# madsjulia/GeostatInversion.jl

Measured on AMD Instinct MI355X. Metric: randSVD GB/s + top-k singular-value rel-err, n=1e6 rank=256, higher is better.
Workload: dtype f64

## Files before the change

### geostatinversion.jl_amd/context.py

```python
import ctypes as C

import numpy as np

from . import _lib as L


class Context:

    def __init__(self, device=0, lib=None):
        self.lib = lib or L.load()
        h = C.c_void_p()
        L.check(self.lib.gsi_ctx_create(C.byref(h), int(device)), self.lib)
        self.h = h
        self.device = int(device)
        self._children = []

    def close(self):
        if getattr(self, "h", None):
            for ch in list(self._children):
                ch.close()
            self.lib.gsi_ctx_destroy(self.h)
            self.h = None

    def __del__(self):
# ... 42 lines not shown

    def phase_times(self):
        ms = (C.c_double * len(L.PHASES))()
        cnt = (C.c_int64 * len(L.PHASES))()
        L.check(self.lib.gsi_ctx_phase_times(self.h, ms, cnt), self.lib)
        return {name: (ms[i], cnt[i]) for i, name in enumerate(L.PHASES)}

    def counters(self):
        out = (C.c_int64 * 4)()
        L.check(self.lib.gsi_ctx_counters(self.h, out), self.lib)
        return {"cholqr2": out[0], "householder": out[1], "jacobi_sweeps": out[2], "scholqr3": out[3]}

    LU_FORMS = ["none", "replicated", "per-step", "persistent-1hop", "persistent-2hop", "persistent-ov"]

    def path_info(self):
        n = 16
        out = (C.c_int64 * n)()
        L.check(self.lib.gsi_ctx_path_info(self.h, out, n), self.lib)
        forms = {self.LU_FORMS[f]: int(out[6 + f]) for f in range(1, 6) if out[6 + f]}
        return {"lu_form": self.LU_FORMS[out[0]] if 0 <= out[0] < 6 else int(out[0]), "lu_forms_run": forms,
                "lu_selftest_mask": int(out[1]), "collectives": int(out[2]), "n_ranks_seen": int(out[3]),
                "lu_timeouts": int(out[4]), "lu_timeouts_recovered": int(out[5]), "svd_sweep_cap_hits": int(out[12]),
                "lowrank_tails": int(out[13]), "lowrank_power_steps": int(out[14]), "lowrank_power_declines": int(out[15])}

    def release_cache(self):
        L.check(self.lib.gsi_ctx_release_cache(self.h), self.lib)

    def device_bytes(self):
        b = C.c_int64()
        L.check(self.lib.gsi_ctx_device_bytes(self.h, C.byref(b)), self.lib)
        return b.value


class _Handle:
    _destroy = None

    def __init__(self, ctx, h):
        self.ctx, self.h = ctx, h
# ... 180 lines not shown
```

### geostatinversion.jl_amd/csrc/api.cpp

```cpp
#include <cmath>
#include <cstdlib>
#include <cstring>
#include <memory>
#include <new>
#include <string>
#include <vector>
#include "../../include/gsi_hip.h"
#include "pipeline.hpp"
#include "pointcov.hpp"

using namespace gsi;

struct gsi_ctx {
  Context c;
};
struct gsi_op {
  Operator op;
};
struct gsi_mat {
  gsi_ctx* ctx;
  Buf buf;
  int64_t rows, cols;
  int refs = 1;
};
// ... 151 lines not shown
  return guarded([&] {
    REQUIRE(ctx && out && n_out >= 1, "bad argument");
    Context& c = ctx->c;
    int64_t v[GSI_PATH_INFO_COUNT] = {0};
    v[GSI_PATH_LU_FORM_LAST] = c.lu_form_last;
    v[GSI_PATH_LU_SELFTEST_MASK] = c.lus_mr_selftest;
    v[GSI_PATH_COLLECTIVES] = c.comm ? c.comm->ncollectives : 0;
    v[GSI_PATH_RANKS_SEEN] = c.ranks_seen;
    v[GSI_PATH_LU_TIMEOUTS] = c.be->lu_timeouts();
    v[GSI_PATH_LU_TIMEOUTS_RECOVERED] = c.lu_timeouts_recovered;
    for (int f = 0; f < (int)Context::LU_FORMS; ++f) v[GSI_PATH_LU_FORM_COUNTS + f] = c.lu_form_count[f];
    v[GSI_PATH_SVD_CAP_HITS] = c.be->svd_cap_hits();
    v[GSI_PATH_LOWRANK_TAILS] = c.lowrank_tails;
    v[GSI_PATH_LOWRANK_POWER_STEPS] = c.lowrank_power_steps;
    v[GSI_PATH_LOWRANK_POWER_DECLINES] = c.lowrank_power_declines;
    for (int64_t i = 0; i < n_out; ++i) out[i] = i < GSI_PATH_INFO_COUNT ? v[i] : 0;
  });
}

int gsi_ctx_pinned_copy_rate(gsi_ctx* ctx, int64_t bytes, double* h2d_gbs, double* d2h_gbs) {
  return guarded([&] {
    REQUIRE(ctx && h2d_gbs && d2h_gbs, "NULL argument");
    REQUIRE(bytes >= 0 && bytes <= ((int64_t)64 << 30), "bad size");
    ctx->c.be->pinned_copy_rate(bytes, h2d_gbs, d2h_gbs);
  });
}

int gsi_ctx_rank(gsi_ctx* ctx, int* rank, int* nranks) {
  return guarded([&] {
    REQUIRE(ctx, "ctx is NULL");
// ... 1053 lines not shown
```

### geostatinversion.jl_amd/csrc/backend.hpp

```cpp
#pragma once
#include <cstddef>
#include <cstdint>
#include <stdexcept>
#include <string>

namespace gsi {

struct Error : std::runtime_error {
  int code;
  Error(int c, const std::string& msg) : std::runtime_error(msg), code(c) {}
};

enum Phase : int {
  PH_GEMM_N = 0, PH_GEMM_T = 1, PH_LU = 2, PH_QR = 3, PH_SVD = 4, PH_SMALL_GEMM = 5,
  PH_COMM = 6, PH_OTHER = 7, PH_COMM_WAIT = 8, PH_COUNT = 9
};

class Backend {
 public:
  virtual ~Backend() {}
  virtual const char* name() const = 0;

  virtual double* alloc(size_t count) = 0;
  virtual void release(double* p) = 0;
// ... 95 lines not shown
  }
  virtual bool sample_gram(const double* S, int64_t ld, int64_t n, int64_t N, double* G) {
    (void)S; (void)ld; (void)n; (void)N; (void)G;
    return false;
  }
  virtual bool lowrank_tail(const double* S, int64_t lds, int64_t n, int64_t N, const double* G, const double* T, int64_t l,
                            int64_t K, double c, double* Z, int64_t ldz, double* Sv) {
    (void)S; (void)lds; (void)n; (void)N; (void)G; (void)T; (void)l; (void)K; (void)c; (void)Z; (void)ldz; (void)Sv;
    return false;
  }
  virtual bool lowrank_power_step(const double* S, int64_t lds, int64_t n, int64_t N, const double* G, const double* T,
                                  const int32_t* ipiv, const double* L, int64_t ldl, int64_t l, double c, double* T_next) {
    (void)S; (void)lds; (void)n; (void)N; (void)G; (void)T; (void)ipiv; (void)L; (void)ldl; (void)l; (void)c; (void)T_next;
    return false;
  }
  virtual void svd_small(double* G, int64_t l, double* U, double* S) = 0;
  virtual void chol_upper(double* B, int64_t j) = 0;
  virtual void trsm_right_upper(double* F, int64_t m, int64_t j, int64_t ldf, const double* C) = 0;

  virtual void scale_cols_sqrt(double* U, int64_t l, const double* S, int64_t K) = 0;
  virtual void center_rows(double* S, int64_t n, int64_t N, int64_t ld) = 0;
  virtual void randn(double* p, size_t count, uint64_t seed) = 0;
  virtual void fill_gridcov(double* A, int64_t lda, int64_t nx, int64_t ny, double ell, int kind,
                            int64_t row0, int64_t mloc) = 0;
  virtual void fill_lowrank_samples(double* S, int64_t ld, int64_t nloc, int64_t N, int64_t row0, uint64_t seed,
                                    double decay) = 0;
  virtual void fftrf_fields(double* dst, int64_t ldd, int64_t row0, int64_t nloc, int64_t nf, int ndims, const int64_t* N,
                            double k0, double dk, double beta, const double* phi, int64_t ldphi, uint64_t seed,
                            int64_t field0) {
    (void)dst; (void)ldd; (void)row0; (void)nloc; (void)nf; (void)ndims; (void)N; (void)k0; (void)dk; (void)beta; (void)phi;
// ... 21 lines not shown
  virtual void lsqr_step_v(int64_t n, const double* t, double* v, double* w, double* x, double* work) = 0;

  virtual void f64_to_f32(const double* src, void* dst32, size_t count) = 0;
  virtual void pcga_params_f32(const void* Z32, int64_t n, int64_t K, const double* s, const double* X, double delta,
                               double* out) = 0;
  virtual void basis_gemv_f32(const void* Z32, int64_t n, int64_t K, const double* w, double beta, const double* X,
                              double* y) = 0;

  virtual int take_error(std::string* msg) = 0;
  virtual bool retryable_failure() { return false; }
  virtual void forgive_lost_coresidency() {}

  virtual void profile(bool on) = 0;
  virtual void phase_begin(Phase p) = 0;
  virtual void phase_end(Phase p) = 0;
  virtual void phase_reset() = 0;
  virtual void phase_times(double* ms, int64_t* counts) = 0;
  virtual void counters(int64_t* out4) { out4[0] = out4[1] = out4[2] = out4[3] = 0; }
  virtual int64_t lu_timeouts() { return 0; }
  virtual int64_t svd_cap_hits() { return 0; }
  virtual void set_ranks_sharing_device(int n) { (void)n; }
};

class Comm {
 public:
  int rank = 0, nranks = 1;
  int64_t ncollectives = 0;
  virtual ~Comm() {}
  void allreduce_sum(double* buf, size_t count) { ++ncollectives; do_allreduce_sum(buf, count); }
  void allgather(const double* send, double* recv, size_t count) { ++ncollectives; do_allgather(send, recv, count); }
// ... 8 lines not shown
  virtual void do_allgather(const double* send, double* recv, size_t count) = 0;
  virtual void do_reduce_scatter_sum(const double* send, double* recv, size_t count) = 0;
  virtual void do_alltoall(const double* send, double* recv, size_t count) = 0;
};

Backend* make_backend(int device_id);
Comm* make_comm(Backend* be, int nranks, int rank, const void* unique_id);
void comm_unique_id(void* id_out);
const char* backend_name();

struct ScopedPhase {
  Backend* be; Phase p;
  ScopedPhase(Backend* b, Phase ph) : be(b), p(ph) { be->phase_begin(p); }
  ~ScopedPhase() { be->phase_end(p); }
};

}
```

### geostatinversion.jl_amd/csrc/hip_backend.hip

```cpp
#include <hip/hip_runtime.h>
#include <rccl/rccl.h>
#include <dlfcn.h>
#include <fcntl.h>
#include <sched.h>
#include <sys/mman.h>
#include <time.h>
#include <unistd.h>
#include <algorithm>
#include <cmath>
#include <cstdlib>
#include <cstring>
#include <condition_variable>
#include <atomic>
#include <mutex>
#include <string>
#include <chrono>
#include <map>
#include <memory>
#include <set>
#include <vector>
#include "../../include/gsi_hip.h"
#include "backend.hpp"
#include "hip_common.hpp"
#include "host_staging.hpp"
// ... 45 lines not shown
    HIP_CHECK(hipGetDeviceProperties(&prop, device_));
    arch_ = prop.gcnArchName;
    ncus_ = prop.multiProcessorCount;
    if (arch_.find("gfx950") == std::string::npos)
      throw Error(GSI_ERR_HIP, "libgsi_hip is built for gfx950 (MI355X); device reports " + arch_);
    HIP_CHECK(hipStreamCreateWithFlags(&st_, hipStreamNonBlocking));
    HIP_CHECK(hipMalloc(&flags_, 16 * sizeof(int32_t)));
    HIP_CHECK(hipMemsetAsync(flags_, 0, 16 * sizeof(int32_t), st_));
    HIP_CHECK(hipMalloc(&scal_, (64 + 8 + 256) * sizeof(double)));
  }
  ~HipBackend() override {
    hipSetDevice(device_);
    hipStreamSynchronize(st_);
    stager_.reset();
    if (ev_stage_) hipEventDestroy(ev_stage_);
    for (auto& b : {&ws_gemm_, &ws_lu_, &ws_qr_, &ws_svd_, &ws_blas2_, &ws_lus_, &ws_svdf_, &ws_qr_hh_}) free_ws(*b);
    collect_garbage();
    for (auto& b : pool_) hipFree(b.p);
    for (auto& ev : ev_pool_) hipEventDestroy(ev);
    for (auto& r : records_) { hipEventDestroy(r.a); hipEventDestroy(r.b); }
    hipFree(flags_);
    hipFree(scal_);
    if (pin_power_) hipHostFree(pin_power_);
    if (mr_recs_) hipFree(mr_recs_);
    hipStreamDestroy(st_);
  }
  const char* name() const override { return "hip-gfx950"; }
  hipStream_t stream() const { return st_; }
  void bind() { hipSetDevice(device_); }

  double* alloc(size_t count) override {
// ... 56 lines not shown
    }
    const int64_t cap = ((int64_t)160 << 30) / std::max(1, ranks_sharing_device_);
    if (pooled_ > cap) trim_pool(cap / 3 * 2);
  }
  void trim_pool(int64_t keep_bytes) {
    hipStreamSynchronize(st_);
    std::lock_guard<std::mutex> g(mu_);
    while (!pool_.empty() && pooled_ > keep_bytes) {
      hipFree(pool_.back().p);
      pooled_ -= (int64_t)pool_.back().bytes;
      pool_.pop_back();
    }
  }
  void release_cache() override {
    bind();
    for (DevBuf* b : {&ws_gemm_, &ws_lu_, &ws_qr_, &ws_svd_, &ws_blas2_, &ws_lus_, &ws_svdf_, &ws_qr_hh_})
      if (b->bytes > ((size_t)64 << 20)) free_ws(*b);
    (void)hipStreamSynchronize(st_);
    collect_garbage();
    trim_pool(0);
  }
  int64_t bytes_in_use() const override {
    int64_t ws = 0;
    for (const DevBuf* b : {&ws_gemm_, &ws_lu_, &ws_qr_, &ws_svd_, &ws_blas2_, &ws_svdf_, &ws_qr_hh_})
      if (!b->pooled) ws += (int64_t)b->bytes;
    return in_use_ + pooled_ + ws + (int64_t)garbage_bytes_;
  }
  HostStager* stager() {
    if (stager_ || stager_failed_) return stager_.get();
    static const int threads = getenv("GSI_STAGE_THREADS") ? std::max(1, std::min(32, atoi(getenv("GSI_STAGE_THREADS")))) : 6;
    static const size_t chunk = (size_t)(getenv("GSI_STAGE_CHUNK_MB") ? std::max(1, std::min(1024, atoi(getenv("GSI_STAGE_CHUNK_MB")))) : 16) << 20;
    try {
      stager_.reset(new HostStager(device_, threads, chunk));
      HIP_CHECK(hipEventCreateWithFlags(&ev_stage_, hipEventDisableTiming));
    } catch (const std::exception&) {
      (void)hipGetLastError();
      stager_.reset();
      stager_failed_ = true;
    }
// ... 845 lines not shown
    const Verdict* h = static_cast<const Verdict*>(pin_power_);
    HIP_CHECK(hipMemcpyAsync(pin_power_, part, sizeof(Verdict), hipMemcpyDeviceToHost, st_));
    HIP_CHECK(hipStreamSynchronize(st_));
    double mx = 0.0;
    bool finite = true;
    for (int p = 0; p < NPARTS; ++p) {
      if (!std::isfinite(h->parts[p])) finite = false;
      else mx = std::max(mx, h->parts[p]);
    }
    if (!finite) mx = INFINITY;
    if (trace) fprintf(stderr, "lowrank_power_step: n %lld N %lld l %lld, %lld moved rows, check max |(P S) C - L| = %.3e\n",
                       (long long)n, (long long)N, (long long)l, (long long)h->v[2], mx);
    if (h->v[0] != 0 || h->v[1] != 0) return false;
    return finite && mx <= CHECK_MAX;
  }
  void svd_small(double* G, int64_t l, double* U, double* S) override {
    bind();
    if (l > 5000) throw Error(GSI_ERR_ARG, "sketch width l = K+p > 5000 is not supported by the LDS-resident block Jacobi SVD");
    grow(ws_svd_, sizeof(double) * (l + 8) + 64 + sizeof(int32_t) * hipk::SVD_SCHED_INTS);
    hipk::SvdWork w;
    w.norms = (double*)ws_svd_.p;
    w.pairs = (int32_t*)((char*)ws_svd_.p + sizeof(double) * (l + 8) + 64);
    w.rotcount = flags_ + 8;
    const int sw = hipk::svd_small(st_, G, l, U, S, w);
    last_svd_sweeps_ = sw < 0 ? -sw : sw;
    if (sw < 0) ++n_svd_cap_hits_;
    check_launch("svd_small");
  }
  void chol_upper(double* B, int64_t j) override {
    bind();
// ... 198 lines not shown
      return GSI_ERR_NOT_POSDEF;
    }
    return 0;
  }

  void profile(bool on) override { prof_ = on; }
  void phase_begin(Phase p) override {
    if (!prof_) return;
    bind();
    if (roctx().push) roctx().push(kPhaseNames[p]);
    cur_.phase = p;
    cur_.a = get_event();
    cur_.b = get_event();
    hipEventRecord(cur_.a, st_);
  }
  void phase_end(Phase) override {
    if (!prof_) return;
    if (roctx().pop) roctx().pop();
    hipEventRecord(cur_.b, st_);
    records_.push_back(cur_);
  }
  void phase_reset() override {
    bind();
    hipStreamSynchronize(st_);
    for (auto& r : records_) { ev_pool_.push_back(r.a); ev_pool_.push_back(r.b); }
    records_.clear();
    for (int i = 0; i < PH_COUNT; ++i) { acc_ms_[i] = 0.0; acc_n_[i] = 0; }
  }
  void phase_times(double* ms, int64_t* counts) override {
    bind();
    hipStreamSynchronize(st_);
    for (auto& r : records_) {
      float t = 0.f;
      if (hipEventElapsedTime(&t, r.a, r.b) == hipSuccess) { acc_ms_[r.phase] += t; acc_n_[r.phase] += 1; }
      ev_pool_.push_back(r.a);
      ev_pool_.push_back(r.b);
    }
    records_.clear();
    for (int i = 0; i < PH_COUNT; ++i) { ms[i] = acc_ms_[i]; counts[i] = acc_n_[i]; }
  }

  void counters(int64_t* out4) override {
    out4[0] = n_cholqr_; out4[1] = n_householder_; out4[2] = last_svd_sweeps_; out4[3] = n_scholqr3_;
  }
  int64_t lu_timeouts() override { return n_lu_timeouts_; }
  int64_t svd_cap_hits() override { return n_svd_cap_hits_; }
  void set_ranks_sharing_device(int n) override { ranks_sharing_device_ = n; }
  int device() const { return device_; }

 private:
  struct Scratch {
    HipBackend* be; double* p;
    Scratch(HipBackend* b, size_t doubles) : be(b), p(doubles ? b->alloc(doubles) : nullptr) {}
    ~Scratch() { if (p) be->release(p); }
    Scratch(const Scratch&) = delete;
    Scratch& operator=(const Scratch&) = delete;
  };
  struct Rec { Phase phase; hipEvent_t a, b; };
  hipEvent_t get_event() {
    if (!ev_pool_.empty()) { hipEvent_t e = ev_pool_.back(); ev_pool_.pop_back(); return e; }
    hipEvent_t e;
    hipEventCreate(&e);
    return e;
  }
  void check_launch(const char* what) {
    hipError_t e = hipGetLastError();
    if (e != hipSuccess) throw Error(GSI_ERR_HIP, std::string(what) + ": " + hipGetErrorString(e));
  }
  void free_ws(DevBuf& b) {
    if (!b.p) return;
    if (b.pooled) release((double*)b.p);
    else { std::lock_guard<std::mutex> g(mu_); garbage_.push_back(b.p); garbage_bytes_ += b.bytes; }
    b.p = nullptr; b.bytes = 0; b.pooled = false;
// ... 38 lines not shown
    if (doubles == 0) return (double*)ws_gemm_.p;
    grow(ws_gemm_, doubles * sizeof(double));
    return (double*)ws_gemm_.p;
  }

  int device_;
  int ncus_ = 0;
  std::string arch_;
  hipStream_t st_ = nullptr;
  std::unique_ptr<HostStager> stager_;
  bool stager_failed_ = false;
  hipEvent_t ev_stage_ = nullptr;
  int32_t* flags_ = nullptr;
  double* scal_ = nullptr;
  void* pin_power_ = nullptr;
  DevBuf ws_gemm_, ws_lu_, ws_qr_, ws_svd_, ws_blas2_, ws_lus_, ws_svdf_, ws_qr_hh_;
  std::mutex mu_;
  std::vector<DevBuf> sizes_;
  std::vector<DevBuf> pool_;
  std::vector<void*> garbage_;
  size_t garbage_bytes_ = 0;
  int64_t in_use_ = 0, pooled_ = 0;
  bool prof_ = false;
  Rec cur_{};
  std::vector<Rec> records_;
  std::vector<hipEvent_t> ev_pool_;
  double acc_ms_[PH_COUNT] = {0};
  int64_t acc_n_[PH_COUNT] = {0};
  int last_svd_sweeps_ = 0;
  int64_t n_svd_cap_hits_ = 0;
  int64_t n_cholqr_ = 0, n_householder_ = 0, n_scholqr3_ = 0;
// ... 470 lines not shown
```

### geostatinversion.jl_amd/csrc/hip_common.hpp

```cpp
#pragma once
#include <hip/hip_runtime.h>
#include <atomic>
#include <cstdint>
#include <cstddef>
#include "pointcov.hpp"

namespace gsi { namespace hipk {

inline bool first_use_on_this_device(std::atomic<uint64_t>& mask) {
  int dev = 0;
  if (hipGetDevice(&dev) != hipSuccess || dev < 0 || dev > 63) return true;
  const uint64_t bit = (uint64_t)1 << dev;
  return (mask.fetch_or(bit, std::memory_order_acq_rel) & bit) == 0;
}

struct GemmPlan { int64_t nt, nchunks, xmode, wide, nsplit, persistent, grid_x, active; };
size_t gemm_workspace_doubles(int64_t M, int64_t L, int64_t K);
void gemm_f64(hipStream_t st, bool transA, int64_t M, int64_t L, int64_t K, double alpha, const double* A,
              int64_t lda, const double* B, int64_t ldb, double beta, double* C, int64_t ldc, double* ws,
              GemmPlan* plan = nullptr);
size_t gemm_rowblock_workspace_doubles(int64_t M_full, int64_t mb, int64_t L, int64_t K);
void gemm_f64_nn_rowblock(hipStream_t st, int64_t M_full, int64_t r0, int64_t mb, int64_t L, int64_t K, const double* A,
                          int64_t lda, const double* B, int64_t ldb, double* C, int64_t ldc, double* ws,
                          GemmPlan* plan = nullptr);
// ... 144 lines not shown
void tri_product(hipStream_t st, const double* R2, const double* R1, int64_t l, double* R);
bool tri_inverse(hipStream_t st, const double* R, int64_t l, double* X);
void lr_gather_rows(hipStream_t st, const double* S, int64_t lds, int64_t N, const int64_t* src, const int64_t* sub,
                    int64_t nr, double* R, int64_t ldr);
void lr_check_rows(hipStream_t st, const double* E, int64_t lde, const double* L, int64_t ldl, const int64_t* rows,
                   int64_t nchk, int64_t l, double* part, int nparts);
void scholqr3_factor(hipStream_t st, const double* Y, int64_t m, int64_t l, int64_t ld, double* T, int64_t ldt,
                     double* S, int64_t lds, double* small_ws, int32_t* flag, double* gemm_ws);
void scholqr3_apply(hipStream_t st, double* Y, int64_t m, int64_t l, int64_t ld, const double* S, int64_t lds,
                    double* R, double* small_ws, double* gemm_ws);

void lr_compose(hipStream_t st, const int32_t* piv, const int32_t* info, int64_t n, int64_t l, int64_t nchk, int64_t o_chk,
                int64_t o_sm, int64_t ldr, int64_t* src, int64_t* sub, int64_t* chk, int32_t* verdict);
void lr_solve_u(hipStream_t st, const double* L, int64_t ldl, const double* Mp, int64_t l, double c, double* Ut);
void lr_solve_c(hipStream_t st, const double* Ut, int64_t l, const double* T, int64_t N, double c, double* C);
struct SvdWork {
  int32_t* rotcount;
  double* norms;
  int32_t* pairs;
};
constexpr int SVD_SCHED_INTS = 4096;
int svd_small(hipStream_t st, double* G, int64_t l, double* U, double* S, const SvdWork& w);

void center_rows(hipStream_t st, double* S, int64_t n, int64_t N, int64_t ld);
void scale_cols_sqrt(hipStream_t st, double* U, int64_t l, const double* S, int64_t K);
void randn_fill(hipStream_t st, double* p, size_t count, uint64_t seed);
void fill_gridcov(hipStream_t st, double* A, int64_t lda, int64_t nx, int64_t ny, double ell, int kind,
                  int64_t row0, int64_t mloc);
void fill_lowrank_samples(hipStream_t st, double* S, int64_t ld, int64_t nloc, int64_t N, int64_t row0, uint64_t seed,
                          double decay);
// ... 25 lines not shown
```

### geostatinversion.jl_amd/csrc/lowrank_power.hip

```cpp
#include "hip_common.hpp"
#include <climits>

namespace gsi { namespace hipk {

constexpr int LRP_MAXL = 384;
constexpr int LRP_THREADS = 256;
constexpr int LRP_ITEMS = 3;

constexpr int LRP_PER = (LRP_MAXL + LRP_THREADS - 1) / LRP_THREADS;

__global__ __launch_bounds__(LRP_THREADS) void lr_compose_kernel(const int32_t* __restrict__ piv, const int32_t* __restrict__ info,
                                                                 int64_t n, int l, int nchk, int64_t o_chk, int64_t o_sm,
                                                                 int64_t ldr, int64_t* __restrict__ src, int64_t* __restrict__ sub,
                                                                 int64_t* __restrict__ chk, int32_t* __restrict__ verdict) {
  __shared__ int32_t top[LRP_MAXL], pv[LRP_MAXL], up[LRP_MAXL], lk[LRP_MAXL], lv[LRP_MAXL], sk[LRP_MAXL], sv[LRP_MAXL];
  __shared__ int32_t scan[LRP_THREADS];
  __shared__ int32_t cnt_s, bad_s;
  const int tid = threadIdx.x;
  if (tid == 0) { cnt_s = 0; bad_s = 0; }
  __syncthreads();
  for (int j = tid; j < l; j += LRP_THREADS) {
    int64_t r = piv[j];
    if (r < j || r >= n) { bad_s = 1; r = r < j ? j : n - 1; }
    pv[j] = (int32_t)r;
// ... 234 lines not shown
    for (int i = lane; i < l; i += 64) C[r0 + cc + (int64_t)i * N] = c * xs[cc][i];
  }
}

constexpr int LRP_NC_U = 2, LRP_NC_C = 4;

void lr_solve_u(hipStream_t st, const double* L, int64_t ldl, const double* Mp, int64_t l, double c, double* Ut) {
  hipLaunchKernelGGL(lr_solve_u_kernel<LRP_NC_U>, dim3((unsigned)((l + LRP_NC_U - 1) / LRP_NC_U)), dim3(64), 0, st, L, ldl, Mp,
                     (int)l, c, Ut);
}
void lr_solve_c(hipStream_t st, const double* Ut, int64_t l, const double* T, int64_t N, double c, double* C) {
  hipLaunchKernelGGL(lr_solve_c_kernel<LRP_NC_C>, dim3((unsigned)((N + LRP_NC_C - 1) / LRP_NC_C)), dim3(64), 0, st, Ut, (int)l, T,
                     N, c, C);
}

}}
```

### geostatinversion.jl_amd/csrc/pipeline.cpp

```cpp
#include "pipeline.hpp"
#include "lsqr_state.hpp"
#include <algorithm>
#include <cmath>
#include <cstdlib>
#include <string>
#include "../../include/gsi_hip.h"

namespace gsi {

void default_shard(int64_t m, int nranks, int rank, int64_t* row0, int64_t* mloc) {
  const int64_t pad = (m + nranks - 1) / nranks;
  int64_t r0 = std::min<int64_t>((int64_t)rank * pad, m);
  *row0 = r0;
  *mloc = std::min<int64_t>(pad, m - r0);
}

void check_async_errors(Context& c) {
  std::string msg;
  const int code = c.be->take_error(&msg);
  if (code != 0) throw Error(code, msg);
}

Operator::~Operator() {
  if (plan && ctx && ctx->be) ctx->be->fftcov_destroy(plan);
// ... 726 lines not shown
  if (A.gram.p != nullptr) return A.gram.p;
  Buf G(be, (size_t)A.N * A.N);
  {
    ScopedPhase ph(be, PH_OTHER);
    if (!be->sample_gram(A.data.p, A.ld, A.mloc, A.N, G.p)) return nullptr;
  }
  A.gram = std::move(G);
  return A.gram.p;
}

static bool lowrank_tail_applies(const Operator& A, int64_t l) {
  static const bool off = (getenv("GSI_NO_LOWRANK_TAIL") != nullptr);
  return !off && A.kind == OP_LOWRANK && !A.ctx->comm && A.m == A.n && A.mloc == A.m && A.N <= 4096 && l <= A.N - 1;
}

static void randsvd_lowrank_single(const Operator& A, const double* Omega, int64_t K, int64_t l, int64_t q, double* Z, double* S) {
  Context& c = *A.ctx;
  Backend* be = c.be.get();
  check_rangefinder_args(A, l, q);
  static const bool power_off = (getenv("GSI_NO_LOWRANK_POWER") != nullptr);
  bool power = !power_off && q > 0;
  const int64_t n = A.n;
  const double cN = 1.0 / (double)(A.N - 1);
  Buf T(be, (size_t)A.N * l), Tn, P;
  if (power) Tn = Buf(be, (size_t)A.N * l);
  int32_t* ipiv = nullptr;
  lowrank_StX(A, Omega, n, l, T.p);
  for (int64_t step = 0; step < 2 * q; ++step) {
    if (P.p == nullptr) P = Buf(be, (size_t)n * l);
    lowrank_ScT(A, T.p, l, P.p, n);
    if (power) {
      ScopedPhase ph(be, PH_LU);
      power = be->lu_L_keep(P.p, n, l, n, &ipiv);
    }
    if (!power) lu_panel(c, P.p, n, l);
    if (power) {
      const double* G = sample_gram(A);
      power = false;
      if (G != nullptr) {
        ScopedPhase ph(be, PH_OTHER);
        power = be->lowrank_power_step(A.data.p, A.ld, A.mloc, A.N, G, T.p, ipiv, P.p, n, l, cN, Tn.p);
        if (!power) c.lowrank_power_declines += 1;
      }
    }
    if (power) {
      std::swap(T, Tn);
      c.lowrank_power_steps += 1;
    } else {
      Tn.reset();
      lowrank_StX(A, P.p, n, l, T.p);
    }
  }
  Tn.reset();
  const double* G = sample_gram(A);
  if (G != nullptr && be->lowrank_tail(A.data.p, A.ld, n, A.N, G, T.p, l, K, cN, Z, n, S)) {
    c.lowrank_tails += 1;
    return;
  }
// ... 191 lines not shown
```

### geostatinversion.jl_amd/csrc/pipeline.hpp

```cpp
#pragma once
#include <cstdint>
#include <functional>
#include <map>
#include <memory>
#include <vector>
#include "backend.hpp"

namespace gsi {

struct Buf {
  Backend* be = nullptr;
  double* p = nullptr;
  size_t count = 0;
  Buf() {}
  Buf(Backend* b, size_t n) : be(b), p(b->alloc(n)), count(n) {}
  Buf(const Buf&) = delete;
  Buf& operator=(const Buf&) = delete;
  Buf(Buf&& o) noexcept : be(o.be), p(o.p), count(o.count) { o.p = nullptr; }
  Buf& operator=(Buf&& o) noexcept {
    if (this != &o) { reset(); be = o.be; p = o.p; count = o.count; o.p = nullptr; }
    return *this;
  }
  ~Buf() { reset(); }
  void reset() { if (p) { be->release(p); p = nullptr; } }
// ... 2 lines not shown
struct Context {
  std::unique_ptr<Backend> be;
  std::unique_ptr<Comm> comm;
  std::map<int64_t, bool> lus_mr_ok;
  int lus_mr_selftest = -1;
  int64_t lus_mr_gen = -1;
  enum LuForm { LU_NONE = 0, LU_REPLICATED = 1, LU_PER_STEP = 2, LU_MR_1HOP = 3, LU_MR_2HOP = 4, LU_MR_OV = 5, LU_FORMS = 6 };
  int64_t lu_form_last = LU_NONE;
  int64_t lu_form_count[LU_FORMS] = {0, 0, 0, 0, 0, 0};
  int64_t ranks_seen = 1;
  int profile_level = 0;
  int64_t lu_timeouts_recovered = 0;
  int64_t lowrank_tails = 0;
  int64_t lowrank_power_steps = 0;
  int64_t lowrank_power_declines = 0;
  int rank() const { return comm ? comm->rank : 0; }
  int nranks() const { return comm ? comm->nranks : 1; }
};

enum OpKind { OP_DENSE = 0, OP_LOWRANK = 1, OP_GRIDCOV_IMPLICIT = 2, OP_FFT_COV = 3, OP_POINTCOV = 4 };

struct Operator {
  Context* ctx = nullptr;
  OpKind kind = OP_DENSE;
  int64_t m = 0, n = 0, row0 = 0, mloc = 0;
  Buf data;
  int64_t ld = 0;
  int64_t N = 0;
  int64_t gx = 0, gy = 0;
  int pc_d = 0, pc_kind = 0;
// ... 47 lines not shown
```

### include/gsi_hip.h

```cpp
#ifndef GSI_HIP_H
#define GSI_HIP_H

#include <stdint.h>

#ifdef __cplusplus
extern "C" {
#endif

#define GSI_VERSION 100

#define GSI_OK 0
#define GSI_ERR_ARG 1
#define GSI_ERR_NEG_ITERS 2
#define GSI_ERR_SINGULAR 3
#define GSI_ERR_HIP 4
#define GSI_ERR_RCCL 5
#define GSI_ERR_OOM 6
#define GSI_ERR_NOT_POSDEF 7
#define GSI_ERR_INTERNAL 8

typedef struct gsi_ctx gsi_ctx;
typedef struct gsi_op gsi_op;
typedef struct gsi_mat gsi_mat;

// ... 144 lines not shown
int gsi_ctx_phase_reset(gsi_ctx* ctx);
int gsi_ctx_phase_times(gsi_ctx* ctx, double* ms_out ,
                        int64_t* count_out );
int gsi_ctx_counters(gsi_ctx* ctx, int64_t* out4);
#define GSI_PATH_LU_FORM_LAST 0
#define GSI_PATH_LU_SELFTEST_MASK 1
#define GSI_PATH_COLLECTIVES 2
#define GSI_PATH_RANKS_SEEN 3
#define GSI_PATH_LU_TIMEOUTS 4
#define GSI_PATH_LU_TIMEOUTS_RECOVERED 5
#define GSI_PATH_LU_FORM_COUNTS 6
#define GSI_PATH_SVD_CAP_HITS 12
#define GSI_PATH_LOWRANK_TAILS 13
#define GSI_PATH_LOWRANK_POWER_STEPS 14
#define GSI_PATH_LOWRANK_POWER_DECLINES 15
#define GSI_PATH_INFO_COUNT 16
int gsi_ctx_path_info(gsi_ctx* ctx, int64_t* out, int64_t n_out);
int gsi_ctx_pinned_copy_rate(gsi_ctx* ctx, int64_t bytes, double* h2d_gbs, double* d2h_gbs);
int gsi_ctx_release_cache(gsi_ctx* ctx);
int gsi_ctx_device_bytes(gsi_ctx* ctx, int64_t* bytes);

#ifdef __cplusplus
}
#endif
#endif
```

Baseline: 1682.

## Split low-rank power-step LU into two column halves with Schur update

In the low-rank randSVD power iteration, the n-by-l panel LU is now factored in two blocks. The first l1=160 columns are factored, then a small Schur-complement update is applied in the N-dimensional sample space before forming and factoring the trailing block. This replaces one wide tall LU with two narrower LUs, which may suit the lu2 kernel better and shrink the GEMM work on the trailing block. It adds several small kernels for pivot composition and row movement, plus a fallback that recomputes the full-width LU when the power step declines.

```diff
diff --git a/geostatinversion.jl_amd/context.py b/geostatinversion.jl_amd/context.py
--- a/geostatinversion.jl_amd/context.py
+++ b/geostatinversion.jl_amd/context.py
@@ -80,14 +80,15 @@
     LU_FORMS = ["none", "replicated", "per-step", "persistent-1hop", "persistent-2hop", "persistent-ov"]
 
     def path_info(self):
-        n = 16
+        n = 18
         out = (C.c_int64 * n)()
         L.check(self.lib.gsi_ctx_path_info(self.h, out, n), self.lib)
         forms = {self.LU_FORMS[f]: int(out[6 + f]) for f in range(1, 6) if out[6 + f]}
         return {"lu_form": self.LU_FORMS[out[0]] if 0 <= out[0] < 6 else int(out[0]), "lu_forms_run": forms,
                 "lu_selftest_mask": int(out[1]), "collectives": int(out[2]), "n_ranks_seen": int(out[3]),
                 "lu_timeouts": int(out[4]), "lu_timeouts_recovered": int(out[5]), "svd_sweep_cap_hits": int(out[12]),
-                "lowrank_tails": int(out[13]), "lowrank_power_steps": int(out[14]), "lowrank_power_declines": int(out[15])}
+                "lowrank_tails": int(out[13]), "lowrank_power_steps": int(out[14]), "lowrank_power_declines": int(out[15]),
+                "lowrank_split_lus": int(out[16]), "lowrank_split_declines": int(out[17])}
 
     def release_cache(self):
         L.check(self.lib.gsi_ctx_release_cache(self.h), self.lib)
diff --git a/geostatinversion.jl_amd/csrc/api.cpp b/geostatinversion.jl_amd/csrc/api.cpp
--- a/geostatinversion.jl_amd/csrc/api.cpp
+++ b/geostatinversion.jl_amd/csrc/api.cpp
@@ -189,6 +189,8 @@
     v[GSI_PATH_LOWRANK_TAILS] = c.lowrank_tails;
     v[GSI_PATH_LOWRANK_POWER_STEPS] = c.lowrank_power_steps;
     v[GSI_PATH_LOWRANK_POWER_DECLINES] = c.lowrank_power_declines;
+    v[GSI_PATH_LOWRANK_SPLIT_LUS] = c.lowrank_split_lus;
+    v[GSI_PATH_LOWRANK_SPLIT_DECLINES] = c.lowrank_split_declines;
     for (int64_t i = 0; i < n_out; ++i) out[i] = i < GSI_PATH_INFO_COUNT ? v[i] : 0;
   });
 }
diff --git a/geostatinversion.jl_amd/csrc/backend.hpp b/geostatinversion.jl_amd/csrc/backend.hpp
--- a/geostatinversion.jl_amd/csrc/backend.hpp
+++ b/geostatinversion.jl_amd/csrc/backend.hpp
@@ -133,6 +133,25 @@
     (void)S; (void)lds; (void)n; (void)N; (void)G; (void)T; (void)ipiv; (void)L; (void)ldl; (void)l; (void)c; (void)T_next;
     return false;
   }
+  virtual bool lowrank_split_ok(int64_t n, int64_t N, int64_t l, int64_t l1) {
+    (void)n; (void)N; (void)l; (void)l1;
+    return false;
+  }
+  virtual void lowrank_split_schur(const double* S, int64_t lds, int64_t n, int64_t N, const double* T, const int32_t* ipiv1,
+                                   const double* P, int64_t ldp, int64_t l, int64_t l1, double c, double* Tt) {
+    (void)S; (void)lds; (void)n; (void)N; (void)T; (void)ipiv1; (void)P; (void)ldp; (void)l; (void)l1; (void)c; (void)Tt;
+    throw Error(1 , "lowrank_split_schur: not available on this backend");
+  }
+  virtual void lowrank_split_rows(double* P, int64_t ldp, int64_t n, int64_t l, int64_t l1) {
+    (void)P; (void)ldp; (void)n; (void)l; (void)l1;
+    throw Error(1 , "lowrank_split_rows: not available on this backend");
+  }
+  virtual void lowrank_split_join(double* P, int64_t ldp, int64_t n, int64_t l, int64_t l1, const int32_t* ipiv2,
+                                  int32_t** ipiv) {
+    (void)P; (void)ldp; (void)n; (void)l; (void)l1; (void)ipiv2; (void)ipiv;
+    throw Error(1 , "lowrank_split_join: not available on this backend");
+  }
+  virtual void lowrank_split_undo() {}
   virtual void svd_small(double* G, int64_t l, double* U, double* S) = 0;
   virtual void chol_upper(double* B, int64_t j) = 0;
   virtual void trsm_right_upper(double* F, int64_t m, int64_t j, int64_t ldf, const double* C) = 0;
@@ -184,6 +203,7 @@
   virtual void profile(bool on) = 0;
   virtual void phase_begin(Phase p) = 0;
   virtual void phase_end(Phase p) = 0;
+  virtual void phase_end_more(Phase p) { phase_end(p); }
   virtual void phase_reset() = 0;
   virtual void phase_times(double* ms, int64_t* counts) = 0;
   virtual void counters(int64_t* out4) { out4[0] = out4[1] = out4[2] = out4[3] = 0; }
@@ -222,5 +242,10 @@
   ScopedPhase(Backend* b, Phase ph) : be(b), p(ph) { be->phase_begin(p); }
   ~ScopedPhase() { be->phase_end(p); }
 };
+struct ScopedPhaseMore {
+  Backend* be; Phase p;
+  ScopedPhaseMore(Backend* b, Phase ph) : be(b), p(ph) { be->phase_begin(p); }
+  ~ScopedPhaseMore() { be->phase_end_more(p); }
+};
 
 }
diff --git a/geostatinversion.jl_amd/csrc/hip_backend.hip b/geostatinversion.jl_amd/csrc/hip_backend.hip
--- a/geostatinversion.jl_amd/csrc/hip_backend.hip
+++ b/geostatinversion.jl_amd/csrc/hip_backend.hip
@@ -83,7 +83,7 @@
     hipStreamSynchronize(st_);
     stager_.reset();
     if (ev_stage_) hipEventDestroy(ev_stage_);
-    for (auto& b : {&ws_gemm_, &ws_lu_, &ws_qr_, &ws_svd_, &ws_blas2_, &ws_lus_, &ws_svdf_, &ws_qr_hh_}) free_ws(*b);
+    for (auto& b : {&ws_gemm_, &ws_lu_, &ws_split_, &ws_qr_, &ws_svd_, &ws_blas2_, &ws_lus_, &ws_svdf_, &ws_qr_hh_}) free_ws(*b);
     collect_garbage();
     for (auto& b : pool_) hipFree(b.p);
     for (auto& ev : ev_pool_) hipEventDestroy(ev);
@@ -170,7 +170,7 @@
   }
   void release_cache() override {
     bind();
-    for (DevBuf* b : {&ws_gemm_, &ws_lu_, &ws_qr_, &ws_svd_, &ws_blas2_, &ws_lus_, &ws_svdf_, &ws_qr_hh_})
+    for (DevBuf* b : {&ws_gemm_, &ws_lu_, &ws_split_, &ws_qr_, &ws_svd_, &ws_blas2_, &ws_lus_, &ws_svdf_, &ws_qr_hh_})
       if (b->bytes > ((size_t)64 << 20)) free_ws(*b);
     (void)hipStreamSynchronize(st_);
     collect_garbage();
@@ -178,7 +178,7 @@
   }
   int64_t bytes_in_use() const override {
     int64_t ws = 0;
-    for (const DevBuf* b : {&ws_gemm_, &ws_lu_, &ws_qr_, &ws_svd_, &ws_blas2_, &ws_svdf_, &ws_qr_hh_})
+    for (const DevBuf* b : {&ws_gemm_, &ws_lu_, &ws_split_, &ws_qr_, &ws_svd_, &ws_blas2_, &ws_svdf_, &ws_qr_hh_})
       if (!b->pooled) ws += (int64_t)b->bytes;
     return in_use_ + pooled_ + ws + (int64_t)garbage_bytes_;
   }
@@ -1054,6 +1054,88 @@
     if (h->v[0] != 0 || h->v[1] != 0) return false;
     return finite && mx <= CHECK_MAX;
   }
+  static constexpr int64_t SPLIT_MAX_L1 = 192;
+  struct SplitWs { int32_t* piv; int32_t* verdict1; int32_t* verdict2; int64_t* idx1; int64_t o_chk, o_sm, ldr; };
+  static int64_t up8(int64_t x) { return (x + 7) & ~(int64_t)7; }
+  SplitWs split_ws(int64_t l1) {
+    SplitWs w;
+    w.o_chk = up8(2 * l1); w.o_sm = w.o_chk + up8(l1); w.ldr = up8(w.o_sm + 2 * l1);
+    grow(ws_split_, 2048 + sizeof(int64_t) * (size_t)(2 * up8(5 * SPLIT_MAX_L1 + 16) + SPLIT_MAX_L1));
+    char* base = (char*)ws_split_.p;
+    w.piv = (int32_t*)base;
+    w.verdict1 = (int32_t*)(base + 1536 + 64);
+    w.verdict2 = w.verdict1 + 4;
+    w.idx1 = (int64_t*)(base + 2048);
+    return w;
+  }
+  bool lu2_takes(int64_t m) {
+    static const bool tall_first = (getenv("GSI_LU_TALL") != nullptr && getenv("GSI_LU_TALL")[0] == '1');
+    hipk::Lu2Work w;
+    return !tall_first && !lu2_lost_ && ranks_sharing_device_ <= 1 && hipk::lu2_config(m, ncus_, &w.bs, &w.rpt, &w.grid) &&
+           lu2_fits(w.bs, w.rpt, w.grid);
+  }
+  bool lowrank_split_ok(int64_t n, int64_t N, int64_t l, int64_t l1) override {
+    bind();
+    if (l1 < 1 || l1 > SPLIT_MAX_L1 || l <= l1 || l > 2 * l1 || l - l1 < 8 || l > 384 || N < 1 || N > 4096 || n < 2 * l ||
+        n >= ((int64_t)1 << 31))
+      return false;
+    return lu2_takes(n) && lu2_takes(n - l1);
+  }
+  void lowrank_split_schur(const double* Sm, int64_t lds, int64_t n, int64_t N, const double* T, const int32_t* ipiv1,
+                           const double* P, int64_t ldp, int64_t l, int64_t l1, double c, double* Tt) override {
+    bind();
+    const int64_t l2 = l - l1;
+    const SplitWs w = split_ws(l1);
+    const size_t l1l = (size_t)up8(l1 * l), Nl1 = (size_t)up8(N * l1);
+    Scratch buf(this, (size_t)up8(l1) * (size_t)N + 2 * l1l + 8 + Nl1);
+    double* R = buf.p;
+    double* Mp = R + (size_t)up8(l1) * N;
+    double* Ut11 = Mp + l1l;
+    double* U12 = Ut11 + (size_t)up8(l1 * l1);
+    double* C1 = Mp + 2 * l1l + 8;
+    size_t gmax = hipk::gemm_workspace_doubles(l1, l, N);
+    gmax = std::max(gmax, hipk::gemm_workspace_doubles(N, l2, l1));
+    double* ws = gemm_ws(gmax + 64);
+    int64_t* src = w.idx1, * sub = w.idx1 + w.ldr, * chk = w.idx1 + 2 * w.ldr;
+    hipk::lr_compose(st_, ipiv1, flags_ + 0, n, l1, l1, w.o_chk, w.o_sm, w.ldr, src, sub, chk, w.verdict1);
+    hipk::lr_pivots(st_, ipiv1, l1, 0, w.piv);
+    hipk::lr_gather_rows(st_, Sm, lds, N, src + w.o_chk, sub + w.o_chk, l1, R, up8(l1));
+    hipk::gemm_f64(st_, false, l1, l, N, 1.0, R, up8(l1), T, N, 0.0, Mp, l1, ws);
+    hipk::lr_solve_u12(st_, P, ldp, Mp, l1, l, c, Ut11, U12);
+    hipk::lr_solve_c(st_, Ut11, l1, T, N, c, C1);
+    hipk::scal_copy(st_, N * l2, c, T + (size_t)N * l1, Tt);
+    hipk::gemm_f64(st_, false, N, l2, l1, -1.0, C1, N, U12, l1, 1.0, Tt, N, ws);
+    check_launch("lowrank_split_schur");
+  }
+  void lowrank_split_rows(double* P, int64_t ldp, int64_t n, int64_t l, int64_t l1) override {
+    bind();
+    (void)n;
+    const int64_t l2 = l - l1;
+    const SplitWs w = split_ws(l1);
+    Scratch tmp(this, (size_t)(2 * l1) * (size_t)l2);
+    hipk::lr_move_rows(st_, P + (size_t)l1 * ldp, ldp, l2, w.idx1, w.idx1 + w.ldr, w.verdict1, 2 * l1, tmp.p, 2 * l1, l1);
+    check_launch("lowrank_split_rows");
+  }
+  void lowrank_split_join(double* P, int64_t ldp, int64_t n, int64_t l, int64_t l1, const int32_t* ipiv2,
+                          int32_t** ipiv) override {
+    bind();
+    const int64_t l2 = l - l1;
+    const SplitWs w = split_ws(l1);
+    const int64_t ldr = up8(4 * l2);
+    Scratch buf(this, (size_t)(2 * ldr + 8) + (size_t)(2 * l2) * (size_t)l1);
+    int64_t* src = reinterpret_cast<int64_t*>(buf.p), * sub = src + ldr, * chk = sub + ldr;
+    double* tmp = buf.p + 2 * ldr + 8;
+    hipk::lr_compose(st_, ipiv2, flags_ + 0, n - l1, l2, 0, 2 * l2, 2 * l2, ldr, src, sub, chk, w.verdict2);
+    hipk::lr_pivots(st_, ipiv2, l2, l1, w.piv + l1);
+    hipk::lr_move_rows(st_, P + l1, ldp, l1, src, sub, w.verdict2, 2 * l2, tmp, 2 * l2, 0);
+    check_launch("lowrank_split_join");
+    *ipiv = w.piv;
+  }
+  void lowrank_split_undo() override {
+    bind();
+    hipk::lr_forget_zero_pivot(st_, flags_ + 0);
+    check_launch("lowrank_split_undo");
+  }
   void svd_small(double* G, int64_t l, double* U, double* S) override {
     bind();
     if (l > 5000) throw Error(GSI_ERR_ARG, "sketch width l = K+p > 5000 is not supported by the LDS-resident block Jacobi SVD");
@@ -1282,10 +1364,13 @@
     cur_.b = get_event();
     hipEventRecord(cur_.a, st_);
   }
-  void phase_end(Phase) override {
+  void phase_end(Phase) override { phase_end_counted(true); }
+  void phase_end_more(Phase) override { phase_end_counted(false); }
+  void phase_end_counted(bool counted) {
     if (!prof_) return;
     if (roctx().pop) roctx().pop();
     hipEventRecord(cur_.b, st_);
+    cur_.counted = counted;
     records_.push_back(cur_);
   }
   void phase_reset() override {
@@ -1300,7 +1385,7 @@
     hipStreamSynchronize(st_);
     for (auto& r : records_) {
       float t = 0.f;
-      if (hipEventElapsedTime(&t, r.a, r.b) == hipSuccess) { acc_ms_[r.phase] += t; acc_n_[r.phase] += 1; }
+      if (hipEventElapsedTime(&t, r.a, r.b) == hipSuccess) { acc_ms_[r.phase] += t; acc_n_[r.phase] += r.counted ? 1 : 0; }
       ev_pool_.push_back(r.a);
       ev_pool_.push_back(r.b);
     }
@@ -1324,7 +1409,7 @@
     Scratch(const Scratch&) = delete;
     Scratch& operator=(const Scratch&) = delete;
   };
-  struct Rec { Phase phase; hipEvent_t a, b; };
+  struct Rec { Phase phase; hipEvent_t a, b; bool counted; };
   hipEvent_t get_event() {
     if (!ev_pool_.empty()) { hipEvent_t e = ev_pool_.back(); ev_pool_.pop_back(); return e; }
     hipEvent_t e;
@@ -1393,7 +1478,7 @@
   int32_t* flags_ = nullptr;
   double* scal_ = nullptr;
   void* pin_power_ = nullptr;
-  DevBuf ws_gemm_, ws_lu_, ws_qr_, ws_svd_, ws_blas2_, ws_lus_, ws_svdf_, ws_qr_hh_;
+  DevBuf ws_gemm_, ws_lu_, ws_split_, ws_qr_, ws_svd_, ws_blas2_, ws_lus_, ws_svdf_, ws_qr_hh_;
   std::mutex mu_;
   std::vector<DevBuf> sizes_;
   std::vector<DevBuf> pool_;
diff --git a/geostatinversion.jl_amd/csrc/hip_common.hpp b/geostatinversion.jl_amd/csrc/hip_common.hpp
--- a/geostatinversion.jl_amd/csrc/hip_common.hpp
+++ b/geostatinversion.jl_amd/csrc/hip_common.hpp
@@ -182,6 +182,12 @@
                 int64_t o_sm, int64_t ldr, int64_t* src, int64_t* sub, int64_t* chk, int32_t* verdict);
 void lr_solve_u(hipStream_t st, const double* L, int64_t ldl, const double* Mp, int64_t l, double c, double* Ut);
 void lr_solve_c(hipStream_t st, const double* Ut, int64_t l, const double* T, int64_t N, double c, double* C);
+void lr_solve_u12(hipStream_t st, const double* L, int64_t ldl, const double* Mp, int64_t l1, int64_t l, double c, double* Ut11,
+                  double* U12);
+void lr_move_rows(hipStream_t st, double* X, int64_t ldx, int64_t nc, const int64_t* src, const int64_t* sub,
+                  const int32_t* verdict, int64_t maxmv, double* tmp, int64_t ldt, int64_t nzero);
+void lr_pivots(hipStream_t st, const int32_t* piv, int64_t cnt, int64_t add, int32_t* dst);
+void lr_forget_zero_pivot(hipStream_t st, int32_t* info);
 struct SvdWork {
   int32_t* rotcount;
   double* norms;
diff --git a/geostatinversion.jl_amd/csrc/lowrank_power.hip b/geostatinversion.jl_amd/csrc/lowrank_power.hip
--- a/geostatinversion.jl_amd/csrc/lowrank_power.hip
+++ b/geostatinversion.jl_amd/csrc/lowrank_power.hip
@@ -272,4 +272,94 @@
                      N, c, C);
 }
 
+template <int NC>
+__global__ __launch_bounds__(64) void lr_solve_u12_kernel(const double* __restrict__ L, int64_t ldl, const double* __restrict__ Mp,
+                                                          int l1, int l, double c, double* __restrict__ Ut11,
+                                                          double* __restrict__ U12) {
+  __shared__ double xs[NC][LRP_MAXL];
+  const int lane = threadIdx.x, col0 = blockIdx.x * NC;
+  const int m = (col0 + NC < l1) ? col0 + NC : l1;
+  double v[NC][LRP_MAXL / 64];
+#pragma unroll
+  for (int cc = 0; cc < NC; ++cc)
+#pragma unroll
+    for (int ib = 0; ib < LRP_MAXL / 64; ++ib) {
+      const int i = ib * 64 + lane;
+      v[cc][ib] = (i < m && col0 + cc < l) ? Mp[i + (int64_t)(col0 + cc) * l1] : 0.0;
+    }
+  __builtin_amdgcn_sched_barrier(0);
+#pragma unroll
+  for (int cc = 0; cc < NC; ++cc)
+#pragma unroll
+    for (int ib = 0; ib < LRP_MAXL / 64; ++ib) xs[cc][ib * 64 + lane] = v[cc][ib];
+  __syncthreads();
+  lrp_lower_solve<NC, true>(L, ldl, m, xs, lane);
+  for (int cc = 0; cc < NC; ++cc) {
+    const int col = col0 + cc;
+    if (col >= l) break;
+    if (col < l1) {
+      for (int i = lane; i <= col; i += 64) Ut11[col + (int64_t)i * l1] = c * xs[cc][i];
+    } else {
+      for (int i = lane; i < l1; i += 64) U12[i + (int64_t)(col - l1) * l1] = c * xs[cc][i];
+    }
+  }
+}
+
+void lr_solve_u12(hipStream_t st, const double* L, int64_t ldl, const double* Mp, int64_t l1, int64_t l, double c, double* Ut11,
+                  double* U12) {
+  hipLaunchKernelGGL(lr_solve_u12_kernel<LRP_NC_U>, dim3((unsigned)((l + LRP_NC_U - 1) / LRP_NC_U)), dim3(64), 0, st, L, ldl, Mp,
+                     (int)l1, (int)l, c, Ut11, U12);
+}
+
+__global__ __launch_bounds__(256) void lr_rows_out_kernel(const double* __restrict__ X, int64_t ldx, int nc,
+                                                          const int64_t* __restrict__ src, const int32_t* __restrict__ verdict,
+                                                          int maxmv, double* __restrict__ tmp, int64_t ldt) {
+  const int nmv = verdict[2] < maxmv ? verdict[2] : maxmv;
+  const int64_t total = (int64_t)nmv * nc;
+  for (int64_t e = (int64_t)blockIdx.x * blockDim.x + threadIdx.x; e < total; e += (int64_t)gridDim.x * blockDim.x) {
+    const int64_t k = e % nmv, c = e / nmv;
+    tmp[k + c * ldt] = X[src[k] + c * ldx];
+  }
+}
+__global__ __launch_bounds__(256) void lr_rows_in_kernel(double* __restrict__ X, int64_t ldx, int nc,
+                                                         const int64_t* __restrict__ sub, const int32_t* __restrict__ verdict,
+                                                         int maxmv, const double* __restrict__ tmp, int64_t ldt, int nzero) {
+  const int nmv = verdict[2] < maxmv ? verdict[2] : maxmv;
+  const int64_t rows = (int64_t)nmv + nzero, total = rows * nc;
+  for (int64_t e = (int64_t)blockIdx.x * blockDim.x + threadIdx.x; e < total; e += (int64_t)gridDim.x * blockDim.x) {
+    const int64_t k = e % rows, c = e / rows;
+    if (k < nmv) {
+      const int64_t r = sub[k];
+      X[r + c * ldx] = r < nzero ? 0.0 : tmp[k + c * ldt];
+    } else {
+      X[(k - nmv) + c * ldx] = 0.0;
+    }
+  }
+}
+
+void lr_move_rows(hipStream_t st, double* X, int64_t ldx, int64_t nc, const int64_t* src, const int64_t* sub,
+                  const int32_t* verdict, int64_t maxmv, double* tmp, int64_t ldt, int64_t nzero) {
+  if (nc < 1 || maxmv < 1) return;
+  const unsigned g_out = (unsigned)((maxmv * nc + 255) / 256), g_in = (unsigned)(((maxmv + nzero) * nc + 255) / 256);
+  hipLaunchKernelGGL(lr_rows_out_kernel, dim3(g_out), dim3(256), 0, st, X, ldx, (int)nc, src, verdict, (int)maxmv, tmp, ldt);
+  hipLaunchKernelGGL(lr_rows_in_kernel, dim3(g_in), dim3(256), 0, st, X, ldx, (int)nc, sub, verdict, (int)maxmv, tmp, ldt,
+                     (int)nzero);
+}
+
+__global__ __launch_bounds__(256) void lr_pivots_kernel(const int32_t* __restrict__ piv, int cnt, int32_t add,
+                                                        int32_t* __restrict__ dst) {
+  const int j = blockIdx.x * blockDim.x + threadIdx.x;
+  if (j < cnt) dst[j] = piv[j] + add;
+}
+void lr_pivots(hipStream_t st, const int32_t* piv, int64_t cnt, int64_t add, int32_t* dst) {
+  hipLaunchKernelGGL(lr_pivots_kernel, dim3((unsigned)((cnt + 255) / 256)), dim3(256), 0, st, piv, (int)cnt, (int32_t)add, dst);
+}
+
+__global__ void lr_forget_zero_pivot_kernel(int32_t* __restrict__ info) {
+  if (info[0] > 0) info[0] = 0;
+}
+void lr_forget_zero_pivot(hipStream_t st, int32_t* info) {
+  hipLaunchKernelGGL(lr_forget_zero_pivot_kernel, dim3(1), dim3(1), 0, st, info);
+}
+
 }}
diff --git a/geostatinversion.jl_amd/csrc/pipeline.cpp b/geostatinversion.jl_amd/csrc/pipeline.cpp
--- a/geostatinversion.jl_amd/csrc/pipeline.cpp
+++ b/geostatinversion.jl_amd/csrc/pipeline.cpp
@@ -764,34 +764,95 @@
   return !off && A.kind == OP_LOWRANK && !A.ctx->comm && A.m == A.n && A.mloc == A.m && A.N <= 4096 && l <= A.N - 1;
 }
 
+static void lowrank_lu_halves(const Operator& A, const double* T, int64_t l, int64_t l1, double* P, double* Tt, int32_t** ipiv) {
+  Backend* be = A.ctx->be.get();
+  const int64_t n = A.n, l2 = l - l1;
+  int32_t* half = nullptr;
+  lowrank_ScT(A, T, l1, P, n);
+  {
+    ScopedPhase ph(be, PH_LU);
+    if (!be->lu_L_keep(P, n, l1, n, &half)) throw Error(GSI_ERR_ARG, "randsvd: lowrank_split_ok without lu_L_keep");
+  }
+  {
+    ScopedPhaseMore ph(be, PH_OTHER);
+    be->lowrank_split_schur(A.data.p, A.ld, n, A.N, T, half, P, n, l, l1, 1.0 / (double)(A.N - 1), Tt);
+  }
+  {
+    ScopedPhaseMore ph(be, PH_GEMM_N);
+    be->gemm_nn(n, l2, A.N, 1.0, A.data.p, A.ld, Tt, A.N, 0.0, P + l1 * n, n);
+  }
+  {
+    ScopedPhaseMore ph(be, PH_OTHER);
+    be->lowrank_split_rows(P, n, n, l, l1);
+  }
+  {
+    ScopedPhaseMore ph(be, PH_LU);
+    if (!be->lu_L_keep(P + l1 + l1 * n, n - l1, l2, n, &half)) throw Error(GSI_ERR_ARG, "randsvd: lowrank_split_ok without lu_L_keep");
+  }
+  {
+    ScopedPhaseMore ph(be, PH_OTHER);
+    be->lowrank_split_join(P, n, n, l, l1, half, ipiv);
+  }
+}
+
 static void randsvd_lowrank_single(const Operator& A, const double* Omega, int64_t K, int64_t l, int64_t q, double* Z, double* S) {
   Context& c = *A.ctx;
   Backend* be = c.be.get();
   check_rangefinder_args(A, l, q);
   static const bool power_off = (getenv("GSI_NO_LOWRANK_POWER") != nullptr);
+  static const bool split_off = (getenv("GSI_NO_LOWRANK_SPLIT") != nullptr);
   bool power = !power_off && q > 0;
   const int64_t n = A.n;
   const double cN = 1.0 / (double)(A.N - 1);
-  Buf T(be, (size_t)A.N * l), Tn, P;
+  constexpr int64_t SPLIT_L1 = 160;
+  bool split = power && !split_off && be->lowrank_split_ok(n, A.N, l, SPLIT_L1);
+  Buf T(be, (size_t)A.N * l), Tn, Tt, P;
   if (power) Tn = Buf(be, (size_t)A.N * l);
+  if (split) Tt = Buf(be, (size_t)A.N * (l - SPLIT_L1));
   int32_t* ipiv = nullptr;
   lowrank_StX(A, Omega, n, l, T.p);
   for (int64_t step = 0; step < 2 * q; ++step) {
     if (P.p == nullptr) P = Buf(be, (size_t)n * l);
-    lowrank_ScT(A, T.p, l, P.p, n);
-    if (power) {
-      ScopedPhase ph(be, PH_LU);
-      power = be->lu_L_keep(P.p, n, l, n, &ipiv);
-    }
-    if (!power) lu_panel(c, P.p, n, l);
+    const bool halves = power && split;
+    if (halves) {
+      lowrank_lu_halves(A, T.p, l, SPLIT_L1, P.p, Tt.p, &ipiv);
+    } else {
+      lowrank_ScT(A, T.p, l, P.p, n);
+      if (power) {
+        ScopedPhase ph(be, PH_LU);
+        power = be->lu_L_keep(P.p, n, l, n, &ipiv);
+      }
+      if (!power) lu_panel(c, P.p, n, l);
+    }
     if (power) {
       const double* G = sample_gram(A);
       power = false;
       if (G != nullptr) {
         ScopedPhase ph(be, PH_OTHER);
         power = be->lowrank_power_step(A.data.p, A.ld, A.mloc, A.N, G, T.p, ipiv, P.p, n, l, cN, Tn.p);
-        if (!power) c.lowrank_power_declines += 1;
       }
+      if (halves && power) c.lowrank_split_lus += 1;
+      if (halves && !power) {
+        c.lowrank_split_declines += 1;
+        split = false;
+        Tt.reset();
+        be->lowrank_split_undo();
+        {
+          ScopedPhaseMore ph(be, PH_GEMM_N);
+          be->gemm_nn(n, l, A.N, cN, A.data.p, A.ld, T.p, A.N, 0.0, P.p, n);
+        }
+        bool whole;
+        {
+          ScopedPhaseMore ph(be, PH_LU);
+          whole = be->lu_L_keep(P.p, n, l, n, &ipiv);
+        }
+        if (!whole) throw Error(GSI_ERR_ARG, "randsvd: lowrank_split_ok without lu_L_keep");
+        if (G != nullptr) {
+          ScopedPhaseMore ph(be, PH_OTHER);
+          power = be->lowrank_power_step(A.data.p, A.ld, A.mloc, A.N, G, T.p, ipiv, P.p, n, l, cN, Tn.p);
+        }
+      }
+      if (!power && G != nullptr) c.lowrank_power_declines += 1;
     }
     if (power) {
       std::swap(T, Tn);
diff --git a/geostatinversion.jl_amd/csrc/pipeline.hpp b/geostatinversion.jl_amd/csrc/pipeline.hpp
--- a/geostatinversion.jl_amd/csrc/pipeline.hpp
+++ b/geostatinversion.jl_amd/csrc/pipeline.hpp
@@ -40,6 +40,8 @@
   int64_t lowrank_tails = 0;
   int64_t lowrank_power_steps = 0;
   int64_t lowrank_power_declines = 0;
+  int64_t lowrank_split_lus = 0;
+  int64_t lowrank_split_declines = 0;
   int rank() const { return comm ? comm->rank : 0; }
   int nranks() const { return comm ? comm->nranks : 1; }
 };
diff --git a/include/gsi_hip.h b/include/gsi_hip.h
--- a/include/gsi_hip.h
+++ b/include/gsi_hip.h
@@ -182,7 +182,9 @@
 #define GSI_PATH_LOWRANK_TAILS 13
 #define GSI_PATH_LOWRANK_POWER_STEPS 14
 #define GSI_PATH_LOWRANK_POWER_DECLINES 15
-#define GSI_PATH_INFO_COUNT 16
+#define GSI_PATH_LOWRANK_SPLIT_LUS 16
+#define GSI_PATH_LOWRANK_SPLIT_DECLINES 17
+#define GSI_PATH_INFO_COUNT 18
 int gsi_ctx_path_info(gsi_ctx* ctx, int64_t* out, int64_t n_out);
 int gsi_ctx_pinned_copy_rate(gsi_ctx* ctx, int64_t bytes, double* h2d_gbs, double* d2h_gbs);
 int gsi_ctx_release_cache(gsi_ctx* ctx);
```

After: 1719, median of 6. 1.02x the previous value.
